# RaghuvirJonnagiri/LatticeBoltzmannSimulations

Measured on AMD Instinct MI355X. Metric: MLUPS (million lattice updates/sec) D2Q9 MRT cavity, higher is better.
Workload: dtype f32

## Files before the change

include/lbm.h:

```cpp
#ifndef LBM_H
#define LBM_H

#include <stddef.h>
#include <stdint.h>

#ifdef __cplusplus
extern "C" {
#endif

#define LBM_ABI_VERSION 4

typedef enum lbm_status {
    LBM_OK = 0,
    LBM_ERR_INVALID = -1,
    LBM_ERR_HIP = -2,
    LBM_ERR_NOMEM = -3,
    LBM_ERR_STATE = -4,
    LBM_ERR_COMM = -5
} lbm_status;

enum { LBM_F32 = 0, LBM_F64 = 1 };
enum { LBM_SRT = 0, LBM_TRT = 1, LBM_MRT = 2 };
enum { LBM_SEM_MRT_PY = 0, LBM_SEM_MRT_GPU = 1,
       LBM_SEM_BOUNCE_BACK = 2 };
// ... 3 lines not shown
       LBM_KERNEL_TB = 3,
       LBM_KERNEL_PUSH = 4,
       LBM_KERNEL_STREAM = 5 };
enum { LBM_LAYOUT_AUTO = 0, LBM_LAYOUT_PLANES = 1, LBM_LAYOUT_ROWS = 2 };
enum { LBM_ARITH_STRICT = 0, LBM_ARITH_FAST = 1, LBM_ARITH_PROMOTED = 2 };
enum { LBM_SIDE_LOW = 0, LBM_SIDE_HIGH = 1 };
enum { LBM_FLAG_NO_DEEP_HALO = 1,
       LBM_FLAG_FRAME_UNFUSED = 2,
       LBM_FLAG_FRAME_FUSED_BATCH = 4,
       LBM_FLAG_NO_FRAME_LDS = 8,
       LBM_FLAG_NT_ON = 16,
       LBM_FLAG_NT_OFF = 32,
       LBM_FLAG_COMM_PRIORITY_OFF = 64,
       LBM_FLAG_EAGER_LAG = 128,
       LBM_FLAG_FRAME_BESIDE_ON = 512,
       LBM_FLAG_FRAME_BESIDE_OFF = 1024,
       LBM_FLAG_FRAME_NARROW = 2048,
       LBM_FLAG_NO_EDGE_FIRST = 4096,
       LBM_FLAG_NO_EDGE_RESERVE = 8192,
       LBM_FLAG_NO_XCD_BANDS = 16384,
       LBM_FLAG_NO_TAIL_TILES = 32768,
       LBM_FLAG_STREAM_WALLS = 65536,
       LBM_FLAG_NO_STREAM_WALLS = 262144,
       LBM_FLAG_STREAM_PAIRS = 131072 };

typedef struct lbm_params {
    int32_t struct_size;
    int32_t nx;
    int32_t ny;
    int32_t y0;
    int32_t ny_local;
    int32_t dtype;
    int32_t collision;
    int32_t semantics;
    int32_t kernel;
    int32_t turb;
    int32_t device;
    int32_t layout;
    int32_t batch;
    int32_t arith;
    int32_t ny_local_min;
    int32_t tb_steps;
    int32_t frame_seg;
    int32_t flags;
    double uLB;
    double omega;
    double omegam;
// ... 56 lines not shown
```

latticeboltzmannsimulations_amd/_lib.py:

```python
import ctypes
import os
import subprocess

_HERE = os.path.dirname(os.path.abspath(__file__))
_CSRC = os.path.join(_HERE, "csrc")
LIB_PATH = os.environ.get("LBM_LIB_PATH", os.path.join(_HERE, "liblbm_hip.so"))
HEADER = os.path.join(os.path.dirname(_HERE), "include", "lbm.h")

HIPCC = os.environ.get("HIPCC", "/opt/rocm/bin/hipcc")
HIPCC_FLAGS = ["--offload-arch=gfx950", "-O3", "-std=c++17", "-ffp-contract=off", "-fPIC", "-shared", "-Wall"]
LINK_FLAGS = ["-ldl"]

LBM_F32, LBM_F64 = 0, 1
LBM_SRT, LBM_TRT, LBM_MRT = 0, 1, 2
LBM_SEM_MRT_PY, LBM_SEM_MRT_GPU, LBM_SEM_BOUNCE_BACK = 0, 1, 2
LBM_KERNEL_AUTO, LBM_KERNEL_GENERIC, LBM_KERNEL_VEC, LBM_KERNEL_TB, LBM_KERNEL_PUSH, LBM_KERNEL_STREAM = 0, 1, 2, 3, 4, 5
LBM_LAYOUT_AUTO, LBM_LAYOUT_PLANES, LBM_LAYOUT_ROWS = 0, 1, 2
LBM_SIDE_LOW, LBM_SIDE_HIGH = 0, 1
LBM_ARITH_STRICT, LBM_ARITH_FAST, LBM_ARITH_PROMOTED = 0, 1, 2
LBM_FLAG_NO_DEEP_HALO, LBM_FLAG_FRAME_UNFUSED, LBM_FLAG_FRAME_FUSED_BATCH, LBM_FLAG_NO_FRAME_LDS = 1, 2, 4, 8
LBM_FLAG_NT_ON, LBM_FLAG_NT_OFF, LBM_FLAG_COMM_PRIORITY_OFF, LBM_FLAG_EAGER_LAG = 16, 32, 64, 128
LBM_FLAG_FRAME_BESIDE_ON, LBM_FLAG_FRAME_BESIDE_OFF, LBM_FLAG_FRAME_NARROW, LBM_FLAG_NO_EDGE_FIRST = 512, 1024, 2048, 4096
LBM_FLAG_NO_EDGE_RESERVE, LBM_FLAG_NO_XCD_BANDS, LBM_FLAG_NO_TAIL_TILES, LBM_FLAG_STREAM_WALLS = 8192, 16384, 32768, 65536
LBM_FLAG_STREAM_PAIRS, LBM_FLAG_NO_STREAM_WALLS = 131072, 262144
ABI_VERSION = 4


class lbm_params(ctypes.Structure):
    _fields_ = [("struct_size", ctypes.c_int32), ("nx", ctypes.c_int32), ("ny", ctypes.c_int32),
                ("y0", ctypes.c_int32), ("ny_local", ctypes.c_int32), ("dtype", ctypes.c_int32),
                ("collision", ctypes.c_int32), ("semantics", ctypes.c_int32), ("kernel", ctypes.c_int32),
                ("turb", ctypes.c_int32), ("device", ctypes.c_int32), ("layout", ctypes.c_int32),
                ("batch", ctypes.c_int32), ("arith", ctypes.c_int32), ("ny_local_min", ctypes.c_int32),
                ("tb_steps", ctypes.c_int32), ("frame_seg", ctypes.c_int32), ("flags", ctypes.c_int32),
                ("uLB", ctypes.c_double), ("omega", ctypes.c_double), ("omegam", ctypes.c_double),
                ("omega_e", ctypes.c_double), ("omega_eps", ctypes.c_double), ("omega_q", ctypes.c_double)]


def sources():
    return [os.path.join(_CSRC, f) for f in sorted(os.listdir(_CSRC)) if f.endswith((".hip", ".hpp"))] + [HEADER]


def build(force=False, verbose=False):
    srcs = sources()
    if not force and os.path.exists(LIB_PATH) and all(os.path.getmtime(LIB_PATH) >= os.path.getmtime(s) for s in srcs):
        return LIB_PATH
    cflags = [f for f in HIPCC_FLAGS if f != "-shared"]
# ... 93 lines not shown
```

latticeboltzmannsimulations_amd/csrc/lbm_host.hpp:

```cpp
#pragma once
#include <hip/hip_runtime.h>
#include <rccl/rccl.h>
#include <dlfcn.h>

#include <algorithm>
#include <chrono>
#include <cstdio>
#include <cstdlib>
#include <cstring>
#include <new>
#include <string>
#include <type_traits>
#include <vector>

#include "../../include/lbm.h"
#include "lbm_inst.hpp"

constexpr int LAT_LAG = 9;
constexpr int NLAT = 10;

enum class Kern { none, tile2, tile, stream, stream_walls, stream_pairs };

struct lbm_ctx {
    lbm_params p{};
// ... 7 lines not shown
    int lag = 0;
    bool lag_valid = false;
    bool lazy_lag = true;
    hipStream_t s_compute = nullptr, s_comm = nullptr;
    hipEvent_t ev_edges = nullptr, ev_halo = nullptr, ev_int = nullptr, ev_go = nullptr, ev_t0 = nullptr, ev_t1 = nullptr;
    void* stage = nullptr;
    size_t stage_bytes = 0;
    double* red_dev = nullptr;
    ncclComm_t comm = nullptr;
    int nranks = 1, rank = 0;
    bool thin_valid = false;
    bool frame_lds = true;
    int frame_seg = 64;
    bool frame_fused = true;
    bool deep_halo = false;
    bool loopback = false;
    bool use_vec = false;
    bool use_nt = false;
    bool push = false;
    Kern kern = Kern::none;
    int edge_rows = 0;
    bool tail_tiles = false;
    bool xcd_bands = true;
    bool edge_reserve = true;
    bool edge_first = true;
    bool frame_wide = true;
    bool frame_beside = false;
    int ncu = 256;
    int tb_steps = 2;
    int tb_f = TB_F;
    int batch = 1;
    long long bstride = 0;
    void* relax_dev = nullptr;
    bool int_stale = false;
    bool edges_pending = false;
    std::string err;
};

namespace lbmhost {

struct rccl_api {
    decltype(&ncclGetUniqueId) GetUniqueId = nullptr;
    decltype(&ncclCommInitRank) CommInitRank = nullptr;
    decltype(&ncclCommDestroy) CommDestroy = nullptr;
    decltype(&ncclGroupStart) GroupStart = nullptr;
    decltype(&ncclGroupEnd) GroupEnd = nullptr;
// ... 110 lines not shown
}
inline int frame_segs(int n, int L) { return (n + L - 1) / L; }
struct StreamPlan { int nstrips, nsegy, H; };

constexpr long long SPIN_US = 3000;
template <typename Q>
bool spin_until_ready(Q&& query) {
    const auto t0 = std::chrono::steady_clock::now();
    for (;;) {
        const hipError_t e = query();
        if (e == hipSuccess) return true;
        if (e != hipErrorNotReady) { (void)hipGetLastError(); return false; }
        if (std::chrono::duration_cast<std::chrono::microseconds>(std::chrono::steady_clock::now() - t0).count() > SPIN_US) return false;
    }
}

inline bool has_neighbour(const lbm_ctx* c, int side) {
    return side == LBM_SIDE_LOW ? c->geo.y0 > 0 : c->geo.y0 + c->geo.ny < c->geo.NY;
}
inline bool is_slab(const lbm_ctx* c) { return has_neighbour(c, LBM_SIDE_LOW) || has_neighbour(c, LBM_SIDE_HIGH); }
inline bool own_transport(const lbm_ctx* c) { return c->comm != nullptr && (c->nranks > 1 || c->loopback); }
inline bool streaming(const lbm_ctx* c) { return c->kern >= Kern::stream; }
inline bool walls_inside(const lbm_ctx* c) { return c->kern >= Kern::stream_walls; }

enum class Route { one_launch, edges_bulk, fused_frame, frame_passes, single_steps };

struct RowBlocks {
    int n = 0;
    char* ptr[Q + 2];
    size_t elems = 0;
};

int ensure_stage(lbm_ctx* c, size_t bytes);
int sync_all(lbm_ctx* c);
int host_to_stage(lbm_ctx* c, const void* host, int host_dtype, int planes);
int stage_to_host(lbm_ctx* c, const void* stage, void* host, int host_dtype, int planes);
bool frame_lds_fits(const lbm_ctx* c, int S, bool deep_rows, int extra = 0, long long budget = FRAME_LDS_BYTES);
int pairs_waves(int S);
StreamPlan plan_stream_on(const lbm_ctx* c, int S, int ncu, long long* cost_out);
StreamPlan plan_stream(const lbm_ctx* c, int S);
bool lag_replayable(const lbm_ctx* c, int S);
int unit_steps(const lbm_ctx* c, int left, bool raw);
Route unit_route(const lbm_ctx* c, int S, bool replay);
std::string validate_params(const lbm_params* p);
lbm_ctx* plan_ctx(const lbm_params* p, int ncu, bool device, std::string& err_out);
int ensure_scratch(lbm_ctx* c, int n);
// ... 27 lines not shown
```

latticeboltzmannsimulations_amd/csrc/lbm_inst.hpp:

```cpp
#pragma once
#include "lbm_stream.hpp"

#define LBM_GPU_VARIANTS(M, R)                                                                                                  \
    M(R, C_SRT, SEM_GPU, false) M(R, C_TRT, SEM_GPU, false) M(R, C_MRT, SEM_GPU, false)                                         \
    M(R, C_MRT_FAST, SEM_GPU, false) M(R, C_SRT_FAST, SEM_GPU, false) M(R, C_TRT_FAST, SEM_GPU, false)                          \
    M(R, C_SRT, SEM_GPU, true) M(R, C_TRT, SEM_GPU, true) M(R, C_MRT, SEM_GPU, true)                                            \
    M(R, C_MRT_FAST, SEM_GPU, true) M(R, C_SRT_FAST, SEM_GPU, true) M(R, C_TRT_FAST, SEM_GPU, true)
#define LBM_PY_VARIANTS(M, R) M(R, C_SRT, SEM_PY, false) M(R, C_TRT, SEM_PY, false) M(R, C_MRT, SEM_PY, false)
#define LBM_BB_VARIANTS(M, R)                                                                                                   \
    M(R, C_SRT, SEM_BB, false) M(R, C_TRT, SEM_BB, false) M(R, C_MRT, SEM_BB, false)                                            \
    M(R, C_MRT_FAST, SEM_BB, false) M(R, C_SRT_FAST, SEM_BB, false) M(R, C_TRT_FAST, SEM_BB, false)
#define LBM_PROM_VARIANTS(M, R)                                                                                                 \
    M(R, C_SRT_PROM, SEM_GPU, false) M(R, C_TRT_PROM, SEM_GPU, false) M(R, C_MRT_PROM, SEM_GPU, false)                          \
    M(R, C_SRT_PROM, SEM_GPU, true) M(R, C_TRT_PROM, SEM_GPU, true) M(R, C_MRT_PROM, SEM_GPU, true)

#define LBM_TILE_ONE(R, COLL, SEM, S, TURB)                                                                                     \
    LBM_X template __global__ void k_stepS_deep<R, COLL, SEM, S, false, TURB>(const R* __restrict__, R* __restrict__, Geo, Relax<R>, Batch<R>, \
                                                                              int, int, int, int, int, FramePtrs<R>, int, int, int, int, int);
#define LBM_TILE_S(R, COLL, SEM, TURB) LBM_TILE_ONE(R, COLL, SEM, 3, TURB) LBM_TILE_ONE(R, COLL, SEM, 4, TURB) LBM_TILE_ONE(R, COLL, SEM, 5, TURB)
#define LBM_STREAM_ONE(R, COLL, SEM, TURB)                                                                                      \
    LBM_X template __global__ void k_stream<R, COLL, SEM, TURB>(const R* __restrict__, R* __restrict__, Geo, Relax<R>, int, int, int, int, int, \
                                                                int, FramePtrs<R>, int, int, int, int, int, int, int, int, int);
#define LBM_STREAMW_ONE(R, COLL, SEM, TURB) \
    LBM_X template __global__ void k_stream_walls<R, COLL, TURB>(const R* __restrict__, R* __restrict__, Geo, Relax<R>, int, int, int, int);
#define LBM_STREAMS_ONE(R, COLL, SEM, TURB)                                                                                     \
    LBM_X template __global__ void k_stream_walls_slab<R, COLL, TURB>(const R* __restrict__, R* __restrict__, Geo, Relax<R>, int, int, int, int, \
                                                                      int, int, int, int, int, int);
#define LBM_STREAMP_ONE(R, COLL, SEM, TURB) \
    LBM_X template __global__ void k_stream_pairs<R, COLL, TURB>(const R* __restrict__, R* __restrict__, Geo, Relax<R>, int, int, int, int);

#define LBM_INST_TILES(R) LBM_GPU_VARIANTS(LBM_TILE_S, R) LBM_PY_VARIANTS(LBM_TILE_S, R)
#define LBM_INST_STREAM(R) LBM_GPU_VARIANTS(LBM_STREAM_ONE, R) LBM_PY_VARIANTS(LBM_STREAM_ONE, R)
#define LBM_INST_STREAMW(R) LBM_GPU_VARIANTS(LBM_STREAMW_ONE, R)
#define LBM_INST_STREAMS(R) LBM_GPU_VARIANTS(LBM_STREAMS_ONE, R)
#define LBM_INST_STREAMP(R) LBM_GPU_VARIANTS(LBM_STREAMP_ONE, R)
#define LBM_INST_TILES_PROM(R) LBM_PROM_VARIANTS(LBM_TILE_S, R)
#define LBM_INST_STREAM_PROM(R) LBM_PROM_VARIANTS(LBM_STREAM_ONE, R) LBM_PROM_VARIANTS(LBM_STREAMW_ONE, R) LBM_PROM_VARIANTS(LBM_STREAMS_ONE, R)
#define LBM_INST_TILES_BB(R) LBM_BB_VARIANTS(LBM_TILE_S, R)
#define LBM_INST_STREAM_BB(R) LBM_BB_VARIANTS(LBM_STREAM_ONE, R)

#ifdef LBM_INST
#define LBM_X
LBM_INST
#else
#define LBM_X extern
LBM_INST_TILES(float) LBM_INST_TILES(double)
LBM_INST_STREAM(float) LBM_INST_STREAM(double)
LBM_INST_STREAMW(float) LBM_INST_STREAMW(double)
LBM_INST_STREAMS(float) LBM_INST_STREAMS(double)
LBM_INST_STREAMP(float) LBM_INST_STREAMP(double)
// ... 5 lines not shown
```

latticeboltzmannsimulations_amd/csrc/lbm_launch.hip:

```cpp
#include "lbm_host.hpp"

namespace lbmhost {

int ensure_scratch(lbm_ctx* c, int n) {
    bool fresh = false;
    for (int i = 2; i < 2 + n && i < LAT_LAG; ++i) {
        if (c->lat[i]) continue;
        hipError_t e = hipMalloc(&c->lat[i], c->lat_bytes);
        if (e != hipSuccess) {
            c->lat[i] = nullptr;
            return fail(c, LBM_ERR_NOMEM, std::string("hipMalloc(scratch lattice of the frame passes): ") + hipGetErrorString(e));
        }
        HIP_TRY(c, hipMemsetAsync(c->lat[i], 0, c->lat_bytes, c->s_compute));
        fresh = true;
    }
    if (fresh) HIP_TRY(c, hipStreamSynchronize(c->s_compute));
    return LBM_OK;
}

int launch_rows(lbm_ctx* c, int from, int to, int row0, int stride, int nrows, hipStream_t s) {
    if (nrows <= 0) return LBM_OK;
    return launch_variant(c, [&](auto v) {
        using VT = decltype(v);
        using R = typename VT::R;
// ... 58 lines not shown
            hipLaunchKernelGGL((k_frame_multi<R, VT::COLL, VT::SEM, VT::TURB, 1024>), dim3(fl.nframe, c->batch), dim3(1024), 0, s, fp, c->geo,
                               relax_of<R>(c->p), batch_of<R>(c), fl.F, S, fl.nsegx, fl.nsegy, lo ? 1 + extra : 0, hi ? 1 + extra : 0, fl.L, 0);
        else
            hipLaunchKernelGGL((k_frame_multi<R, VT::COLL, VT::SEM, VT::TURB, BLK>), dim3(fl.nframe, c->batch), dim3(BLK), 0, s, fp, c->geo,
                               relax_of<R>(c->p), batch_of<R>(c), fl.F, S, fl.nsegx, fl.nsegy, lo ? 1 + extra : 0, hi ? 1 + extra : 0, fl.L,
                               fl.in_lds ? 1 : 0);
    });
}

static int launch_k_stream(lbm_ctx* c, int from, int to, hipStream_t s, int S, const FrameLayout& fl, const StreamPlan& pl, int nseg, int ye,
                           int lo, int hi, int bands, bool xcd_bands) {
    return launch_variant(c, [&](auto v) {
        using VT = decltype(v);
        using R = typename VT::R;
        hipLaunchKernelGGL((k_stream<R, VT::COLL, VT::SEM, VT::TURB>), dim3(fl.nframe + pl.nstrips * nseg), dim3(ST_NT), 0, s, (const R*)c->lat[from],
                           (R*)c->lat[to], c->geo, relax_of<R>(c->p), S, fl.F, c->geo.nx - fl.F, ye, pl.nstrips, pl.H, frame_ptrs<R>(c, from, to, S),
                           fl.nframe, fl.nsegx, fl.nsegy, fl.L, fl.in_lds ? 1 : 0, lo, hi, bands, xcd_bands ? 1 : 0);
    });
}

static int launch_walls(lbm_ctx* c, int from, int to, hipStream_t s, int S, int ybeg, int yend, int bands, int elo, int ehi) {
    const StreamPlan pl = plan_stream(c, S);
    const int xcd = c->xcd_bands ? 1 : 0;
    return launch_variant(c, [&](auto v) {
        using VT = decltype(v);
        using R = typename VT::R;
        if constexpr (VT::SEM == SEM_GPU) {
            const R* src = (const R*)c->lat[from];
            R* dst = (R*)c->lat[to];
            if (is_slab(c))
                hipLaunchKernelGGL((k_stream_walls_slab<R, VT::COLL, VT::TURB>), dim3(pl.nstrips * (bands ? (bands & 1) + (bands >> 1) : pl.nsegy)),
                                   dim3(ST_NT), 0, s, src, dst, c->geo, relax_of<R>(c->p), S, pl.nstrips, pl.H, bands ? 0 : xcd, ybeg, yend, bands,
                                   elo, ehi, bands ? c->tb_f : 0);
            else if constexpr (coll_is_prom(VT::COLL)) {
                hipLaunchKernelGGL((k_stream_walls<R, VT::COLL, VT::TURB>), dim3(pl.nstrips * pl.nsegy), dim3(ST_NT), 0, s, src, dst, c->geo,
                                   relax_of<R>(c->p), S, pl.nstrips, pl.H, xcd);
            } else if (c->kern == Kern::stream_pairs)
                hipLaunchKernelGGL((k_stream_pairs<R, VT::COLL, VT::TURB>), dim3(pl.nstrips * pl.nsegy), dim3(64 * pairs_waves(S)), 0, s, src, dst,
                                   c->geo, relax_of<R>(c->p), S, pl.nstrips, pl.H, xcd);
            else
                hipLaunchKernelGGL((k_stream_walls<R, VT::COLL, VT::TURB>), dim3(pl.nstrips * pl.nsegy), dim3(ST_NT), 0, s, src, dst, c->geo,
                                   relax_of<R>(c->p), S, pl.nstrips, pl.H, xcd);
        }
    });
}

int launch_stream(lbm_ctx* c, int from, int to, hipStream_t s, int S, bool with_frame) {
    const int F = c->tb_f, ny = c->geo.ny;
    if (walls_inside(c)) {
        const bool slab = is_slab(c);
        if (slab == with_frame) return fail(c, LBM_ERR_STATE, "internal: the streaming kernel with the walls inside takes a whole lone lattice or a slab's bulk rows");
        return launch_walls(c, from, to, s, S, has_neighbour(c, LBM_SIDE_LOW) ? F : 0, ny - (has_neighbour(c, LBM_SIDE_HIGH) ? F : 0), 0, 0, 0);
    }
    FrameLayout fl;
    const int rc = frame_layout(c, fl, S, F, ny - F, ST_LDS_BYTES, false, 0, with_frame);
    if (rc) return rc;
    const StreamPlan pl = plan_stream(c, S);
    return launch_k_stream(c, from, to, s, S, fl, pl, pl.nsegy, ny - F, 0, 0, 0, c->xcd_bands);
}

int launch_stream_edges(lbm_ctx* c, int from, int to, hipStream_t s, int S, bool lo, bool hi, int extra) {
    const int elo = lo ? 1 + extra : 0, ehi = hi ? 1 + extra : 0, bands = (lo ? 1 : 0) | (hi ? 2 : 0);
    if (walls_inside(c)) return launch_walls(c, from, to, s, S, 0, 0, bands, elo, ehi);
    const int F = c->tb_f, ny = c->geo.ny;
    FrameLayout fl;
// ... 316 lines not shown
```

latticeboltzmannsimulations_amd/csrc/lbm_plan.hip:

```cpp
#include "lbm_host.hpp"

namespace lbmhost {

bool frame_lds_fits(const lbm_ctx* c, int S, bool deep_rows, int extra, long long budget) {
    if (!c->frame_lds) return false;
    const int F = c->tb_f, L = c->frame_seg, m = S - 1, np = c->p.turb ? Q + 2 : Q;
    const long long row_strip = (long long)(L + 2 * m + 2) * (F + m + (deep_rows ? m + extra : 0) + 2);
    const long long col_strip = (long long)(F + m + 2) * (L + 2 * m + extra + 2);
    return 2 * np * std::max(row_strip, col_strip) * c->es <= budget;
}
int pairs_waves(int S) { return std::min(SP_MAX_WAVES, S + 2); }
StreamPlan plan_stream_on(const lbm_ctx* c, int S, int ncu, long long* cost_out) {
    const bool walls = walls_inside(c);
    const int V = 16 / c->es, Rr = stream_rim(S, V), TXu = 64 * V - 2 * Rr, F = walls ? 0 : c->tb_f;
    const int cols = c->geo.nx - 2 * F;
    const int rows = walls ? c->geo.ny - c->tb_f * ((has_neighbour(c, LBM_SIDE_LOW) ? 1 : 0) + (has_neighbour(c, LBM_SIDE_HIGH) ? 1 : 0))
                           : c->geo.ny - 2 * F;
    StreamPlan best{walls ? stream_walls_strips(c->geo.nx, S, V) : (cols + TXu - 1) / TXu, 1, rows};
    long long best_cost = -1;
    for (int n = 1; n <= 256 && n * 8 <= std::max(rows, 8); ++n) {
        const int H = (rows + n - 1) / n, nseg = (rows + H - 1) / H;
        const long long segs = (long long)best.nstrips * nseg, rounds = (segs + ncu - 1) / ncu;
        long long iters = H + 2 * (S - 1) + ST_WAVES - 1;
        if (c->kern == Kern::stream_pairs) {
// ... 150 lines not shown
    if (p->kernel == LBM_KERNEL_STREAM && !can_stream)
        return "kernel = STREAM takes one lattice (no batch) with nx % (16 / sizeof(real)) == 0, nx >= 64, ny_local >= 64 (on every rank)";
    const long long cells_plan = (long long)p->nx * nyp;
    const bool walls_variant = c->batch == 1 && !slab && p->semantics == LBM_SEM_MRT_GPU && !p->turb && !(p->flags & LBM_FLAG_NO_STREAM_WALLS) &&
                               (p->collision == LBM_MRT || p->collision == LBM_SRT);
    const bool walls_pays = walls_variant && (c->es == 8 ? p->nx >= 1024 && cells_plan >= (1LL << 20)
                                                         : (p->nx >= 4096 && cells_plan >= (2LL << 20)) || (p->nx >= 2048 && cells_plan >= (4LL << 20)));
    const bool stream_pays = walls_pays ||
                             (p->nx >= 2048 ? (slab ? cells_plan >= (1LL << 20) && nyp >= 512 : cells_plan >= ((c->es == 8 ? 4LL : 8LL) << 20))
                                            : cells_plan >= 3072LL * 3072);
    if (!can_stream || !(p->kernel == LBM_KERNEL_STREAM || (p->kernel == LBM_KERNEL_AUTO && stream_pays))) {
        c->kern = can_tb && (p->kernel == LBM_KERNEL_TB || (p->kernel == LBM_KERNEL_AUTO && big)) ? Kern::tile : Kern::none;
        return std::string();
    }
    const int forced = p->flags & (LBM_FLAG_STREAM_WALLS | LBM_FLAG_STREAM_PAIRS);
    const bool walls_ok = c->batch == 1 && p->semantics == LBM_SEM_MRT_GPU && (!slab || !(p->flags & LBM_FLAG_NO_DEEP_HALO));
    bool walls_pay = !p->turb && (p->collision == LBM_MRT || p->collision == LBM_SRT);
    if (walls_ok && walls_pay && device && !forced) {
        dispatch(c->p, [&](auto v) {
            using VT = decltype(v);
            using R = typename VT::R;
            if constexpr (VT::SEM == SEM_GPU) {
                hipFuncAttributes at;
                const void* kern = slab ? reinterpret_cast<const void*>(&k_stream_walls_slab<R, VT::COLL, VT::TURB>)
                                        : reinterpret_cast<const void*>(&k_stream_walls<R, VT::COLL, VT::TURB>);
                if (hipFuncGetAttributes(&at, kern) != hipSuccess || at.localSizeBytes > (p->collision == LBM_SRT ? 128u : 64u))
                    walls_pay = false;
            }
        });
    }
    const bool walls = walls_ok && !(p->flags & LBM_FLAG_NO_STREAM_WALLS) && (walls_pay || forced);
    c->kern = !walls ? Kern::stream : !slab && (p->flags & LBM_FLAG_STREAM_PAIRS) ? Kern::stream_pairs : Kern::stream_walls;
    return std::string();
}

static std::string plan_steps(lbm_ctx* c) {
    const lbm_params* p = &c->p;
    const int nyp = ny_plan(p);
    if (streaming(c)) {
        c->tb_steps = p->tb_steps ? p->tb_steps : ST_MAX_S;
        const int fmin = p->semantics == LBM_SEM_MRT_PY ? 1 : 0;
        c->tb_f = (c->tb_steps + fmin + 3) / 4 * 4;
        while (c->tb_steps > 2 && (p->nx < 2 * c->tb_f + 16 || nyp < 2 * c->tb_f + 16)) {
            c->tb_steps -= 1;
            c->tb_f = (c->tb_steps + fmin + 3) / 4 * 4;
        }
        if (c->kern == Kern::stream_pairs) c->tb_steps = p->tb_steps ? p->tb_steps : 10;
        else if (c->tb_steps > ST_MAX_S)
            return "tb_steps " + std::to_string(ST_MAX_S + 1) + " .. " + std::to_string(SP_MAX_S) + " need the streaming kernel with two rows per wave (a lone lattice, MRT_GPU semantics)";
        if (c->kern == Kern::stream_walls && is_slab(c) && c->tb_steps < 3) c->kern = Kern::stream;
// ... 32 lines not shown
    }
    c->frame_fused = !(p->flags & LBM_FLAG_FRAME_UNFUSED);
    c->frame_lds = !(p->flags & LBM_FLAG_NO_FRAME_LDS);
    c->frame_wide = !(p->flags & LBM_FLAG_FRAME_NARROW);
    if ((c->frame_seg = p->frame_seg)) return;
    const long long cells1 = (long long)p->nx * ny_plan(p) * c->batch;
    c->frame_seg = cells1 <= 512LL * 512 ? 16 : (cells1 <= 1024LL * 1024 ? 32 : 64);
    if (c->kern == Kern::tile && c->frame_fused && !is_slab(c) && c->frame_lds)
        while (c->frame_seg > 16 && !frame_lds_fits(c, c->tb_steps, false, 0, TILE_FRAME_LDS_BYTES)) c->frame_seg -= 8;
    if (streaming(c) && c->frame_lds)
        while (c->frame_seg > 16 && !frame_lds_fits(c, c->tb_steps, false, 1, ST_LDS_BYTES)) c->frame_seg -= 8;
    if (c->frame_beside) {
        const long long per = 2LL * p->nx + 2LL * (ny_plan(p) - 2 * c->tb_f);
        c->frame_seg = std::max(64, (int)(((per + c->ncu - 1) / c->ncu + 7) / 8 * 8));
    }
}

lbm_ctx* plan_ctx(const lbm_params* p, int ncu, bool device, std::string& err_out) {
    lbm_ctx* c = new (std::nothrow) lbm_ctx();
    if (!c) return (err_out = "out of host memory", nullptr);
    c->p = *p;
    c->ncu = ncu;
    plan_geometry(c);
    err_out = plan_kernel(c, device);
    if (err_out.empty()) err_out = plan_steps(c);
    if (!err_out.empty()) return (delete c, nullptr);
    plan_frame(c, device);
    c->edge_first = !(p->flags & LBM_FLAG_NO_EDGE_FIRST);
    c->edge_reserve = !(p->flags & LBM_FLAG_NO_EDGE_RESERVE);
    c->xcd_bands = !(p->flags & LBM_FLAG_NO_XCD_BANDS);
    c->deep_halo = p->semantics == LBM_SEM_MRT_GPU && !(p->flags & LBM_FLAG_NO_DEEP_HALO);
    c->use_nt = (p->flags & LBM_FLAG_NT_ON) ? true : (p->flags & LBM_FLAG_NT_OFF) ? false : (c->lat_bytes > ((size_t)192 << 20));
    c->lazy_lag = !(p->flags & LBM_FLAG_EAGER_LAG);
    return c;
}

}

using namespace lbmhost;

extern "C" {

int lbm_next_unit(const lbm_ctx* c, int steps_left) {
    if (!c || steps_left < 0) return LBM_ERR_INVALID;
    if (c->push) return steps_left > 0 ? 1 : 0;
    return unit_steps(c, steps_left, c->raw[c->cur] != 0);
// ... 62 lines not shown
```

latticeboltzmannsimulations_amd/csrc/lbm_stream.hpp:

```cpp
#pragma once
#include "lbm_kernels.hpp"

constexpr int ST_WAVES = 16;
constexpr int ST_NT = ST_WAVES * 64;
constexpr int ST_MAX_S = ST_WAVES / 2;
constexpr int ST_LDS_BYTES = ST_WAVES * 9 * 1024;

__device__ __forceinline__ int dpp_from_lower(int v) { return __builtin_amdgcn_update_dpp(v, v, 0x138, 0xf, 0xf, false); }
__device__ __forceinline__ int dpp_from_upper(int v) { return __builtin_amdgcn_update_dpp(v, v, 0x130, 0xf, 0xf, false); }
__device__ __forceinline__ float lane_lower(float v) { return __builtin_bit_cast(float, dpp_from_lower(__builtin_bit_cast(int, v))); }
__device__ __forceinline__ float lane_upper(float v) { return __builtin_bit_cast(float, dpp_from_upper(__builtin_bit_cast(int, v))); }
__device__ __forceinline__ double lane_lower(double v) {
    const long long b = __builtin_bit_cast(long long, v);
    const unsigned lo = (unsigned)dpp_from_lower((int)(unsigned)b), hi = (unsigned)dpp_from_lower((int)(unsigned)(b >> 32));
    return __builtin_bit_cast(double, (long long)(((unsigned long long)hi << 32) | lo));
}
__device__ __forceinline__ double lane_upper(double v) {
    const long long b = __builtin_bit_cast(long long, v);
    const unsigned lo = (unsigned)dpp_from_upper((int)(unsigned)b), hi = (unsigned)dpp_from_upper((int)(unsigned)(b >> 32));
    return __builtin_bit_cast(double, (long long)(((unsigned long long)hi << 32) | lo));
}

__device__ __forceinline__ float lane_lower_e(float v, float edge) {
    return __builtin_bit_cast(float, __builtin_amdgcn_update_dpp(__builtin_bit_cast(int, edge), __builtin_bit_cast(int, v), 0x138, 0xf, 0xf, false));
// ... 118 lines not shown
                                         typename VecT<R, V>::type o3, typename VecT<R, V>::type u2, typename VecT<R, V>::type u5,
                                         typename VecT<R, V>::type u6, typename VecT<R, V>::type d4, typename VecT<R, V>::type d7,
                                         typename VecT<R, V>::type d8) {
    in[0] = o0;
    in[2] = u2;
    in[4] = d4;
    if (WALLS) {
        in[1] = shift_from_lower_e<R, V>(o1, (R)0 + o3[1]);
        in[5] = shift_from_lower_e<R, V>(u5, (R)0 + d7[1]);
        in[8] = shift_from_lower_e<R, V>(d8, (R)0 + u6[1]);
        in[3] = shift_from_upper_e<R, V>(o3, (R)0 + o1[V - 2]);
        in[6] = shift_from_upper_e<R, V>(u6, (R)0 + d8[V - 2]);
        in[7] = shift_from_upper_e<R, V>(d7, (R)0 + u5[V - 2]);
    } else {
        in[1] = shift_from_lower<R, V>(o1);
        in[5] = shift_from_lower<R, V>(u5);
        in[8] = shift_from_lower<R, V>(d8);
        in[3] = shift_from_upper<R, V>(o3);
        in[6] = shift_from_upper<R, V>(u6);
        in[7] = shift_from_upper<R, V>(d7);
    }
}

template <typename R, int COLL, bool TURB, bool WALLS = false, bool SLAB = false>
__device__ __forceinline__ void stream_segment(const R* __restrict__ src, R* __restrict__ dst, const Geo& geo, const Relax<R>& w, R* __restrict__ lds,
                                               int S, int xs, int ya, int yb, int xe, int own_lo = 0, int own_hi = 0) {
    constexpr int V = 16 / (int)sizeof(R), ROW = 64 * V;
    typedef typename VecT<R, V>::type T;
    const int wv = __builtin_amdgcn_readfirstlane((int)(threadIdx.x >> 6)), lane = threadIdx.x & 63;
    const int q = ((wv & 7) << 1) | (wv >> 3);
    const int RV = stream_rim(S, V) / V;
    const bool wall_lo = WALLS && (!SLAB || geo.y0 == 0), wall_hi = WALLS && (!SLAB || geo.y0 + geo.ny == geo.NY);
    const int y_first = wall_lo ? max(ya - (S - 1), 0) : ya - (S - 1);
    const int y_end = wall_hi ? min(yb + (S - 1), geo.ny) : yb + (S - 1);
    const int y_lid = wall_lo ? 0 : -(1 << 30), y_bot = wall_hi ? geo.ny - 1 : -(1 << 30);
    const int nb = y_end - y_first;
    const int x0 = xs + lane * V;
    const bool lane_in = x0 < geo.nx;
    const bool lane_out = WALLS ? (x0 >= own_lo && x0 < own_hi) : (lane >= RV && lane < 64 - RV && x0 < xe);
    const bool wl = WALLS && x0 == 0, wr = WALLS && x0 + V == geo.nx;
    const bool side_strip = WALLS && (xs == 0 || xs + ROW >= geo.nx);
    const bool narrow = WALLS && xs + ROW > geo.nx;
    R* const slot_mine = lds + (q * 9) * ROW;
    R* const up_mine = slot_mine + lane * V;
    const R* const up_below = lds + (((q + 1) & (ST_WAVES - 1)) * 9) * ROW + lane * V;
    const R* const down_above = lds + (((q + ST_WAVES - 1) & (ST_WAVES - 1)) * 9 + 3) * ROW + lane * V;

    T in[Q], outv[Q], hq, hr;
#ifdef LBM_EXP_NO_HBM
    auto row_base = [&](const R* p, int k, int y) { return (const char*)(p + ((long long)k * geo.plane + (long long)((y & 63) + GHY) * geo.row)); };
#else
    auto row_base = [&](const R* p, int k, int y) { return (const char*)(p + ((long long)k * geo.plane + (long long)(y + GHY) * geo.row)); };
#endif
    const unsigned lane_off = (unsigned)(GH + x0) * (unsigned)sizeof(R);
    auto cell = [&](const char* base, int dx) {
        unsigned off = lane_off;
        asm volatile("" : "+v"(off));
        return (const R*)(base + (off + (unsigned)(dx * (int)sizeof(R))));
    };
    const unsigned lane_off_ld = WALLS ? (unsigned)(GH + min(x0, max(geo.nx - V, 0))) * (unsigned)sizeof(R) : lane_off;
    auto cell_ld = [&](const char* base, int dx) {
        unsigned off = lane_off_ld;
        asm volatile("" : "+v"(off));
        return (const R*)(base + (off + (unsigned)(dx * (int)sizeof(R))));
    };
    auto load_row = [&](int y, bool exists) {
        if (WALLS) {
            if (exists) {
#pragma unroll
// ... 105 lines not shown
                if (lid) rw_done = *reinterpret_cast<const T*>(st + lane * V);
                kl_done = st[ROW + lane];
                kr_done = st[2 * ROW + lane];
            }
            if (lane_out && y >= ya && y < yb) {
#pragma unroll
                for (int k = 0; k < Q; ++k) vstore<R, V, false>(const_cast<R*>(cell(row_base(dst, k, y), 0)), outv[k]);
                if (TURB) {
                    vstore<R, V, false>(const_cast<R*>(cell(row_base(dst, K_QEQ, y), 0)), hq_done);
                    vstore<R, V, false>(const_cast<R*>(cell(row_base(dst, K_RHO, y), 0)), hr_done);
                }
                if (WALLS && wrow) {
                    if (lid) {
                        vstore<R, V, false>(const_cast<R*>(cell(row_base(dst, 0, -1), 0)), rw_done);
                        if (wl) *const_cast<R*>(cell(row_base(dst, 7, -1), 1)) = kl_done;
                        if (wr) *const_cast<R*>(cell(row_base(dst, 8, -1), V - 2)) = kr_done;
                    } else {
                        if (wl) *const_cast<R*>(cell(row_base(dst, 6, geo.ny), 1)) = kl_done;
                        if (wr) *const_cast<R*>(cell(row_base(dst, 5, geo.ny), V - 2)) = kr_done;
                    }
                }
            }
            if (S > 1) lds_barrier();
            load_row(y_first + b + ST_WAVES, b + ST_WAVES < nb);
            if (S > 1) lds_barrier();
        }
        for (int i = 2 * S; i < ST_WAVES; ++i) lds_barrier();
    };
#pragma unroll
    for (int k = 0; k < Q; ++k) in[k] = T{};
    hq = T{}; hr = T{};
    for (int i = 0; i < q; ++i) lds_barrier();
    load_row(y_first + q, q < nb);
    for (int b = q; b < nb; b += ST_WAVES) {
        const int y = y_first + b;
        if (WALLS && (SLAB ? (y == y_lid || y == y_bot) : (y == 0 || y == geo.ny - 1))) block(b, std::true_type{});
        else block(b, std::false_type{});
    }
}

template <typename R, int COLL, int SEM, bool TURB>
__global__ __launch_bounds__(ST_NT) void k_stream(const R* __restrict__ src, R* __restrict__ dst, Geo geo, Relax<R> w, int S, int F, int xe, int ye,
                                                  int nstrips, int H, FramePtrs<R> fp, int nframe, int nsegx, int nsegy, int seg, int use_lds,
                                                  int lo, int hi, int bands, int xcd_bands) {
    __shared__ __align__(16) R lds[ST_LDS_BYTES / sizeof(R)];
    if ((int)blockIdx.x < nframe) {
        frame_passes<R, COLL, SEM, TURB, ST_NT>(fp, 0, geo, w, F, S, nsegx, nsegy, lo, hi, (int)blockIdx.x, seg, use_lds ? lds : nullptr, bands);
        return;
    }
    constexpr int V = 16 / (int)sizeof(R);
    int b = blockIdx.x - nframe;
    if (xcd_bands) {
        const int per = ((int)gridDim.x - nframe) >> 3;
        if (b < (per << 3)) b = (b & 7) * per + (b >> 3);
    }
    const int strip = b % nstrips, sy = b / nstrips;
    const int R_ = stream_rim(S, V);
// ... 1 lines not shown
    int ya, yb;
    if (bands) {
        const bool top = (bands & 1) && sy == 0;
        if (top) { ya = -(lo > 0 ? lo - 1 : 0); yb = F; }
        else { ya = geo.ny - F; yb = geo.ny + (hi > 0 ? hi - 1 : 0); }
    } else {
        ya = F + sy * H; yb = min(ye, ya + H);
    }
    if (ya >= yb) return;
    stream_segment<R, COLL, TURB>(src, dst, geo, w, lds, S, xs, ya, yb, xe);
}

__host__ __device__ constexpr int stream_walls_strips(int nx, int S, int V) {
    return nx <= 64 * V ? 1 : (nx - 64 * V + (64 * V - 2 * stream_rim(S, V)) - 1) / (64 * V - 2 * stream_rim(S, V)) + 1;
}
template <int V>
__device__ __forceinline__ void walls_strip(const Geo& geo, int S, int strip, int nstrips, int& xs, int& own_lo, int& own_hi) {
    const int R_ = stream_rim(S, V), TXu = 64 * V - 2 * R_;
    xs = min(strip * TXu, max(geo.nx - 64 * V, 0));
    own_lo = strip == 0 ? 0 : strip * TXu + R_;
    own_hi = strip == nstrips - 1 ? geo.nx : (strip + 1) * TXu + R_;
}

template <typename R, int COLL, bool TURB>
__global__ __launch_bounds__(ST_NT) void k_stream_walls(const R* __restrict__ src, R* __restrict__ dst, Geo geo, Relax<R> w, int S, int nstrips, int H,
                                                        int xcd_bands) {
    __shared__ __align__(16) R lds[ST_LDS_BYTES / sizeof(R)];
    constexpr int V = 16 / (int)sizeof(R);
    const int b = xcd_bands ? xcd_band(blockIdx.x, gridDim.x) : (int)blockIdx.x;
    const int strip = b % nstrips, sy = b / nstrips;
    int xs, own_lo, own_hi;
    walls_strip<V>(geo, S, strip, nstrips, xs, own_lo, own_hi);
    const int ya = sy * H, yb = min(geo.ny, ya + H);
    if (ya >= yb) return;
    stream_segment<R, COLL, TURB, true>(src, dst, geo, w, lds, S, xs, ya, yb, 0, own_lo, own_hi);
}
template <typename R, int COLL, bool TURB>
__global__ __launch_bounds__(ST_NT) void k_stream_walls_slab(const R* __restrict__ src, R* __restrict__ dst, Geo geo, Relax<R> w, int S, int nstrips, int H,
                                                             int xcd_bands, int ybeg, int yend, int bands, int lo, int hi, int F) {
    __shared__ __align__(16) R lds[ST_LDS_BYTES / sizeof(R)];
    constexpr int V = 16 / (int)sizeof(R), W = 64 * V;
    int b = blockIdx.x;
    if (xcd_bands) {
        const int per = (int)gridDim.x >> 3;
        if (b < (per << 3)) b = (b & 7) * per + (b >> 3);
    }
    const int strip = b % nstrips, sy = b / nstrips;
    const int R_ = stream_rim(S, V), TXu = W - 2 * R_;
    const int xs = min(strip * TXu, max(geo.nx - W, 0));
    const int own_lo = strip == 0 ? 0 : strip * TXu + R_;
    const int own_hi = strip == nstrips - 1 ? geo.nx : (strip + 1) * TXu + R_;
    int ya, yb;
    if (bands) {
        const bool top = (bands & 1) && sy == 0;
        if (top) { ya = -(lo > 0 ? lo - 1 : 0); yb = F; }
        else { ya = geo.ny - F; yb = geo.ny + (hi > 0 ? hi - 1 : 0); }
    } else {
        ya = ybeg + sy * H; yb = min(yend, ya + H);
    }
    if (ya >= yb) return;
    stream_segment<R, COLL, TURB, true, true>(src, dst, geo, w, lds, S, xs, ya, yb, 0, own_lo, own_hi);
}

constexpr int SP_MAX_WAVES = 12;
constexpr int SP_NT = SP_MAX_WAVES * 64;

constexpr int SP_MAX_S = SP_MAX_WAVES - 2;
constexpr int SP_SLOTS = 12;
constexpr int SP_LDS_BYTES = SP_MAX_WAVES * SP_SLOTS * 1024;

template <typename R, int COLL, bool TURB>
__device__ __forceinline__ void stream_pairs_segment(const R* __restrict__ src, R* __restrict__ dst, const Geo& geo, const Relax<R>& w, R* __restrict__ lds,
                                                     int S, int xs, int ya, int yb, int own_lo, int own_hi) {
    constexpr int V = 16 / (int)sizeof(R), ROW = 64 * V;
    typedef typename VecT<R, V>::type T;
    const int W = (int)(blockDim.x >> 6);
    const int wv = __builtin_amdgcn_readfirstlane((int)(threadIdx.x >> 6)), lane = threadIdx.x & 63;
    const int y_first = max(ya - (S - 1), 0), y_end = min(yb + (S - 1), geo.ny);
    const int nb = y_end - y_first, npairs = (nb + 1) >> 1;
    const int x0 = xs + lane * V;
    const bool lane_out = x0 >= own_lo && x0 < own_hi;
    const bool wl = x0 == 0, wr = x0 + V == geo.nx;
    const bool side_strip = xs == 0 || xs + ROW >= geo.nx;
    const bool narrow = xs + ROW > geo.nx;
// ... 201 lines not shown
```

latticeboltzmannsimulations_amd/solver.py:

```python
import ctypes

import numpy as np

from . import _lib as L

_DT = {np.dtype(np.float32): L.LBM_F32, np.dtype(np.float64): L.LBM_F64}
_COLL = {"SRT": L.LBM_SRT, "TRT": L.LBM_TRT, "MRT": L.LBM_MRT}
_SEM = {"mrt_py": L.LBM_SEM_MRT_PY, "mrt_gpu": L.LBM_SEM_MRT_GPU, "bounce_back": L.LBM_SEM_BOUNCE_BACK}
_KERNEL = {"auto": L.LBM_KERNEL_AUTO, "generic": L.LBM_KERNEL_GENERIC, "vec": L.LBM_KERNEL_VEC, "tb": L.LBM_KERNEL_TB,
           "push": L.LBM_KERNEL_PUSH, "stream": L.LBM_KERNEL_STREAM}
_ARITH = {"strict": L.LBM_ARITH_STRICT, "fast": L.LBM_ARITH_FAST, "promoted": L.LBM_ARITH_PROMOTED}
_LAYOUT = {"auto": L.LBM_LAYOUT_AUTO, "planes": L.LBM_LAYOUT_PLANES, "rows": L.LBM_LAYOUT_ROWS}


def relaxation(Re, ysize, uLB=0.08, omega_eps=1.2, omega_q=1.2):
    nuLB = uLB * ysize / Re
    omega = 2.0 / (6. * nuLB + 1)
    delTRT = 1.0 / 3.5
    omegam = 1.0 / (0.5 + (delTRT / ((1 / omega) - 0.5)))
    return dict(omega=omega, omegam=omegam, omega_e=1.0, omega_eps=omega_eps, omega_q=omega_q)


def _tuning(t):
    t = dict(t or {})
    tb, seg, flags = int(t.pop("tb_steps", 0) or 0), int(t.pop("frame_seg", 0) or 0), 0
    off = {"deep_halo": L.LBM_FLAG_NO_DEEP_HALO, "frame_fused": L.LBM_FLAG_FRAME_UNFUSED, "frame_lds": L.LBM_FLAG_NO_FRAME_LDS,
           "comm_priority": L.LBM_FLAG_COMM_PRIORITY_OFF, "frame_wide": L.LBM_FLAG_FRAME_NARROW, "edge_first": L.LBM_FLAG_NO_EDGE_FIRST,
           "edge_reserve": L.LBM_FLAG_NO_EDGE_RESERVE, "xcd_bands": L.LBM_FLAG_NO_XCD_BANDS,
           "tail_tiles": L.LBM_FLAG_NO_TAIL_TILES}
    on = {"frame_fused_batch": L.LBM_FLAG_FRAME_FUSED_BATCH, "eager_lag": L.LBM_FLAG_EAGER_LAG, "stream_pairs": L.LBM_FLAG_STREAM_PAIRS}
    if "stream_walls" in t:
        flags |= L.LBM_FLAG_STREAM_WALLS if t.pop("stream_walls") else L.LBM_FLAG_NO_STREAM_WALLS
    for k, bit in off.items():
        if not t.pop(k, True):
            flags |= bit
    for k, bit in on.items():
        if t.pop(k, False):
            flags |= bit
    nt = t.pop("nt", None)
    if nt is not None:
        flags |= L.LBM_FLAG_NT_ON if nt else L.LBM_FLAG_NT_OFF
    fb = t.pop("frame_beside", None)
    if fb is not None:
        flags |= L.LBM_FLAG_FRAME_BESIDE_ON if fb else L.LBM_FLAG_FRAME_BESIDE_OFF
    if t:
        raise ValueError(f"unknown tuning switches {sorted(t)}")
    return tb, seg, flags


class CavitySolver:

    def __init__(self, xsize, ysize, Re, RT="MRT", uLB=0.08, semantics="mrt_gpu", dtype=np.float32, turb=0,
# ... 288 lines not shown
```

Baseline: 374,800.

## Split stream-walls workgroup into two independent wave rings for short time units

Adds a SPLIT template variant of the wall-aware streaming kernels. It divides the 16 waves of a workgroup into two independent 8-wave pipelines, each handling half of the row segment with its own LDS region and ring indexing. The variant is used by default when the temporal-blocking depth S is small (2*S fits within the stage limit). The aim is to cut ring fill/drain barriers and idle waves for short units. The cost is more halo rows recomputed per half-segment and extra kernel instantiations, and the variant is dropped if it spills.

```diff
diff --git a/include/lbm.h b/include/lbm.h
--- a/include/lbm.h
+++ b/include/lbm.h
@@ -49,7 +49,8 @@
        LBM_FLAG_NO_TAIL_TILES = 32768,
        LBM_FLAG_STREAM_WALLS = 65536,
        LBM_FLAG_NO_STREAM_WALLS = 262144,
-       LBM_FLAG_STREAM_PAIRS = 131072 };
+       LBM_FLAG_STREAM_PAIRS = 131072,
+       LBM_FLAG_NO_SHORT_SPLIT = 524288 };
 
 typedef struct lbm_params {
     int32_t struct_size;
diff --git a/latticeboltzmannsimulations_amd/_lib.py b/latticeboltzmannsimulations_amd/_lib.py
--- a/latticeboltzmannsimulations_amd/_lib.py
+++ b/latticeboltzmannsimulations_amd/_lib.py
@@ -22,7 +22,7 @@
 LBM_FLAG_NT_ON, LBM_FLAG_NT_OFF, LBM_FLAG_COMM_PRIORITY_OFF, LBM_FLAG_EAGER_LAG = 16, 32, 64, 128
 LBM_FLAG_FRAME_BESIDE_ON, LBM_FLAG_FRAME_BESIDE_OFF, LBM_FLAG_FRAME_NARROW, LBM_FLAG_NO_EDGE_FIRST = 512, 1024, 2048, 4096
 LBM_FLAG_NO_EDGE_RESERVE, LBM_FLAG_NO_XCD_BANDS, LBM_FLAG_NO_TAIL_TILES, LBM_FLAG_STREAM_WALLS = 8192, 16384, 32768, 65536
-LBM_FLAG_STREAM_PAIRS, LBM_FLAG_NO_STREAM_WALLS = 131072, 262144
+LBM_FLAG_STREAM_PAIRS, LBM_FLAG_NO_STREAM_WALLS, LBM_FLAG_NO_SHORT_SPLIT = 131072, 262144, 524288
 ABI_VERSION = 4
 
 
diff --git a/latticeboltzmannsimulations_amd/csrc/lbm_host.hpp b/latticeboltzmannsimulations_amd/csrc/lbm_host.hpp
--- a/latticeboltzmannsimulations_amd/csrc/lbm_host.hpp
+++ b/latticeboltzmannsimulations_amd/csrc/lbm_host.hpp
@@ -53,6 +53,7 @@
     int edge_rows = 0;
     bool tail_tiles = false;
     bool xcd_bands = true;
+    bool short_split = true;
     bool edge_reserve = true;
     bool edge_first = true;
     bool frame_wide = true;
@@ -209,6 +210,7 @@
 inline bool own_transport(const lbm_ctx* c) { return c->comm != nullptr && (c->nranks > 1 || c->loopback); }
 inline bool streaming(const lbm_ctx* c) { return c->kern >= Kern::stream; }
 inline bool walls_inside(const lbm_ctx* c) { return c->kern >= Kern::stream_walls; }
+inline bool split_unit(const lbm_ctx* c, int S) { return c->kern == Kern::stream_walls && c->short_split && S >= 2 && 2 * S <= ST_MAX_S; }
 
 enum class Route { one_launch, edges_bulk, fused_frame, frame_passes, single_steps };
 
diff --git a/latticeboltzmannsimulations_amd/csrc/lbm_inst.hpp b/latticeboltzmannsimulations_amd/csrc/lbm_inst.hpp
--- a/latticeboltzmannsimulations_amd/csrc/lbm_inst.hpp
+++ b/latticeboltzmannsimulations_amd/csrc/lbm_inst.hpp
@@ -21,11 +21,13 @@
 #define LBM_STREAM_ONE(R, COLL, SEM, TURB)                                                                                      \
     LBM_X template __global__ void k_stream<R, COLL, SEM, TURB>(const R* __restrict__, R* __restrict__, Geo, Relax<R>, int, int, int, int, int, \
                                                                 int, FramePtrs<R>, int, int, int, int, int, int, int, int, int);
-#define LBM_STREAMW_ONE(R, COLL, SEM, TURB) \
-    LBM_X template __global__ void k_stream_walls<R, COLL, TURB>(const R* __restrict__, R* __restrict__, Geo, Relax<R>, int, int, int, int);
-#define LBM_STREAMS_ONE(R, COLL, SEM, TURB)                                                                                     \
-    LBM_X template __global__ void k_stream_walls_slab<R, COLL, TURB>(const R* __restrict__, R* __restrict__, Geo, Relax<R>, int, int, int, int, \
-                                                                      int, int, int, int, int, int);
+#define LBM_STREAMW_SPLIT(R, COLL, SEM, TURB, SPLIT) \
+    LBM_X template __global__ void k_stream_walls<R, COLL, TURB, SPLIT>(const R* __restrict__, R* __restrict__, Geo, Relax<R>, int, int, int, int);
+#define LBM_STREAMS_SPLIT(R, COLL, SEM, TURB, SPLIT)                                                                            \
+    LBM_X template __global__ void k_stream_walls_slab<R, COLL, TURB, SPLIT>(const R* __restrict__, R* __restrict__, Geo, Relax<R>, int, int, int, \
+                                                                             int, int, int, int, int, int, int);
+#define LBM_STREAMW_ONE(R, COLL, SEM, TURB) LBM_STREAMW_SPLIT(R, COLL, SEM, TURB, false) LBM_STREAMW_SPLIT(R, COLL, SEM, TURB, true)
+#define LBM_STREAMS_ONE(R, COLL, SEM, TURB) LBM_STREAMS_SPLIT(R, COLL, SEM, TURB, false) LBM_STREAMS_SPLIT(R, COLL, SEM, TURB, true)
 #define LBM_STREAMP_ONE(R, COLL, SEM, TURB) \
     LBM_X template __global__ void k_stream_pairs<R, COLL, TURB>(const R* __restrict__, R* __restrict__, Geo, Relax<R>, int, int, int, int);
 
diff --git a/latticeboltzmannsimulations_amd/csrc/lbm_launch.hip b/latticeboltzmannsimulations_amd/csrc/lbm_launch.hip
--- a/latticeboltzmannsimulations_amd/csrc/lbm_launch.hip
+++ b/latticeboltzmannsimulations_amd/csrc/lbm_launch.hip
@@ -104,25 +104,26 @@
 static int launch_walls(lbm_ctx* c, int from, int to, hipStream_t s, int S, int ybeg, int yend, int bands, int elo, int ehi) {
     const StreamPlan pl = plan_stream(c, S);
     const int xcd = c->xcd_bands ? 1 : 0;
+    const bool split = split_unit(c, S);
     return launch_variant(c, [&](auto v) {
         using VT = decltype(v);
         using R = typename VT::R;
         if constexpr (VT::SEM == SEM_GPU) {
             const R* src = (const R*)c->lat[from];
             R* dst = (R*)c->lat[to];
-            if (is_slab(c))
-                hipLaunchKernelGGL((k_stream_walls_slab<R, VT::COLL, VT::TURB>), dim3(pl.nstrips * (bands ? (bands & 1) + (bands >> 1) : pl.nsegy)),
-                                   dim3(ST_NT), 0, s, src, dst, c->geo, relax_of<R>(c->p), S, pl.nstrips, pl.H, bands ? 0 : xcd, ybeg, yend, bands,
-                                   elo, ehi, bands ? c->tb_f : 0);
-            else if constexpr (coll_is_prom(VT::COLL)) {
-                hipLaunchKernelGGL((k_stream_walls<R, VT::COLL, VT::TURB>), dim3(pl.nstrips * pl.nsegy), dim3(ST_NT), 0, s, src, dst, c->geo,
-                                   relax_of<R>(c->p), S, pl.nstrips, pl.H, xcd);
-            } else if (c->kern == Kern::stream_pairs)
-                hipLaunchKernelGGL((k_stream_pairs<R, VT::COLL, VT::TURB>), dim3(pl.nstrips * pl.nsegy), dim3(64 * pairs_waves(S)), 0, s, src, dst,
-                                   c->geo, relax_of<R>(c->p), S, pl.nstrips, pl.H, xcd);
-            else
-                hipLaunchKernelGGL((k_stream_walls<R, VT::COLL, VT::TURB>), dim3(pl.nstrips * pl.nsegy), dim3(ST_NT), 0, s, src, dst, c->geo,
-                                   relax_of<R>(c->p), S, pl.nstrips, pl.H, xcd);
+            if (is_slab(c)) {
+                auto kern = split ? k_stream_walls_slab<R, VT::COLL, VT::TURB, true> : k_stream_walls_slab<R, VT::COLL, VT::TURB, false>;
+                hipLaunchKernelGGL(kern, dim3(pl.nstrips * (bands ? (bands & 1) + (bands >> 1) : pl.nsegy)), dim3(ST_NT), 0, s, src, dst, c->geo,
+                                   relax_of<R>(c->p), S, pl.nstrips, pl.H, bands ? 0 : xcd, ybeg, yend, bands, elo, ehi, bands ? c->tb_f : 0);
+            } else if (c->kern == Kern::stream_pairs) {
+                if constexpr (!coll_is_prom(VT::COLL))
+                    hipLaunchKernelGGL((k_stream_pairs<R, VT::COLL, VT::TURB>), dim3(pl.nstrips * pl.nsegy), dim3(64 * pairs_waves(S)), 0, s, src,
+                                       dst, c->geo, relax_of<R>(c->p), S, pl.nstrips, pl.H, xcd);
+            } else {
+                auto kern = split ? k_stream_walls<R, VT::COLL, VT::TURB, true> : k_stream_walls<R, VT::COLL, VT::TURB, false>;
+                hipLaunchKernelGGL(kern, dim3(pl.nstrips * pl.nsegy), dim3(ST_NT), 0, s, src, dst, c->geo, relax_of<R>(c->p), S, pl.nstrips,
+                                   pl.H, xcd);
+            }
         }
     });
 }
diff --git a/latticeboltzmannsimulations_amd/csrc/lbm_plan.hip b/latticeboltzmannsimulations_amd/csrc/lbm_plan.hip
--- a/latticeboltzmannsimulations_amd/csrc/lbm_plan.hip
+++ b/latticeboltzmannsimulations_amd/csrc/lbm_plan.hip
@@ -196,10 +196,15 @@
             using R = typename VT::R;
             if constexpr (VT::SEM == SEM_GPU) {
                 hipFuncAttributes at;
-                const void* kern = slab ? reinterpret_cast<const void*>(&k_stream_walls_slab<R, VT::COLL, VT::TURB>)
-                                        : reinterpret_cast<const void*>(&k_stream_walls<R, VT::COLL, VT::TURB>);
-                if (hipFuncGetAttributes(&at, kern) != hipSuccess || at.localSizeBytes > (p->collision == LBM_SRT ? 128u : 64u))
+                const void* kern = slab ? reinterpret_cast<const void*>(&k_stream_walls_slab<R, VT::COLL, VT::TURB, false>)
+                                        : reinterpret_cast<const void*>(&k_stream_walls<R, VT::COLL, VT::TURB, false>);
+                const void* kern_split = slab ? reinterpret_cast<const void*>(&k_stream_walls_slab<R, VT::COLL, VT::TURB, true>)
+                                              : reinterpret_cast<const void*>(&k_stream_walls<R, VT::COLL, VT::TURB, true>);
+                const size_t bound = p->collision == LBM_SRT ? 128u : 64u;
+                if (hipFuncGetAttributes(&at, kern) != hipSuccess || at.localSizeBytes > bound)
                     walls_pay = false;
+                if (hipFuncGetAttributes(&at, kern_split) != hipSuccess || at.localSizeBytes > bound)
+                    c->short_split = false;
             }
         });
     }
@@ -278,6 +283,7 @@
     c->p = *p;
     c->ncu = ncu;
     plan_geometry(c);
+    c->short_split = !(p->flags & LBM_FLAG_NO_SHORT_SPLIT);
     err_out = plan_kernel(c, device);
     if (err_out.empty()) err_out = plan_steps(c);
     if (!err_out.empty()) return (delete c, nullptr);
diff --git a/latticeboltzmannsimulations_amd/csrc/lbm_stream.hpp b/latticeboltzmannsimulations_amd/csrc/lbm_stream.hpp
--- a/latticeboltzmannsimulations_amd/csrc/lbm_stream.hpp
+++ b/latticeboltzmannsimulations_amd/csrc/lbm_stream.hpp
@@ -164,19 +164,25 @@
     }
 }
 
-template <typename R, int COLL, bool TURB, bool WALLS = false, bool SLAB = false>
+template <typename R, int COLL, bool TURB, bool WALLS = false, bool SLAB = false, bool SPLIT = false>
 __device__ __forceinline__ void stream_segment(const R* __restrict__ src, R* __restrict__ dst, const Geo& geo, const Relax<R>& w, R* __restrict__ lds,
                                                int S, int xs, int ya, int yb, int xe, int own_lo = 0, int own_hi = 0) {
     constexpr int V = 16 / (int)sizeof(R), ROW = 64 * V;
+    constexpr int P = SPLIT ? ST_WAVES / 2 : ST_WAVES;
     typedef typename VecT<R, V>::type T;
     const int wv = __builtin_amdgcn_readfirstlane((int)(threadIdx.x >> 6)), lane = threadIdx.x & 63;
-    const int q = ((wv & 7) << 1) | (wv >> 3);
+    const int q = SPLIT ? ((wv & 3) << 1) | ((wv >> 2) & 1) : ((wv & 7) << 1) | (wv >> 3);
+    if constexpr (SPLIT) {
+        const int ym = ya + ((yb - ya + 1) >> 1);
+        if (wv >> 3) { ya = ym; lds += (P * 9) * ROW; }
+        else yb = ym;
+    }
     const int RV = stream_rim(S, V) / V;
     const bool wall_lo = WALLS && (!SLAB || geo.y0 == 0), wall_hi = WALLS && (!SLAB || geo.y0 + geo.ny == geo.NY);
     const int y_first = wall_lo ? max(ya - (S - 1), 0) : ya - (S - 1);
     const int y_end = wall_hi ? min(yb + (S - 1), geo.ny) : yb + (S - 1);
     const int y_lid = wall_lo ? 0 : -(1 << 30), y_bot = wall_hi ? geo.ny - 1 : -(1 << 30);
-    const int nb = y_end - y_first;
+    const int nb = !SPLIT || ya < yb ? y_end - y_first : 0;
     const int x0 = xs + lane * V;
     const bool lane_in = x0 < geo.nx;
     const bool lane_out = WALLS ? (x0 >= own_lo && x0 < own_hi) : (lane >= RV && lane < 64 - RV && x0 < xe);
@@ -185,8 +191,8 @@
     const bool narrow = WALLS && xs + ROW > geo.nx;
     R* const slot_mine = lds + (q * 9) * ROW;
     R* const up_mine = slot_mine + lane * V;
-    const R* const up_below = lds + (((q + 1) & (ST_WAVES - 1)) * 9) * ROW + lane * V;
-    const R* const down_above = lds + (((q + ST_WAVES - 1) & (ST_WAVES - 1)) * 9 + 3) * ROW + lane * V;
+    const R* const up_below = lds + (((q + 1) & (P - 1)) * 9) * ROW + lane * V;
+    const R* const down_above = lds + (((q + P - 1) & (P - 1)) * 9 + 3) * ROW + lane * V;
 
     T in[Q], outv[Q], hq, hr;
 #ifdef LBM_EXP_NO_HBM
@@ -338,17 +344,17 @@
                 }
             }
             if (S > 1) lds_barrier();
-            load_row(y_first + b + ST_WAVES, b + ST_WAVES < nb);
+            load_row(y_first + b + P, b + P < nb);
             if (S > 1) lds_barrier();
         }
-        for (int i = 2 * S; i < ST_WAVES; ++i) lds_barrier();
+        for (int i = 2 * S; i < P; ++i) lds_barrier();
     };
 #pragma unroll
     for (int k = 0; k < Q; ++k) in[k] = T{};
     hq = T{}; hr = T{};
     for (int i = 0; i < q; ++i) lds_barrier();
     load_row(y_first + q, q < nb);
-    for (int b = q; b < nb; b += ST_WAVES) {
+    for (int b = q; b < nb; b += P) {
         const int y = y_first + b;
         if (WALLS && (SLAB ? (y == y_lid || y == y_bot) : (y == 0 || y == geo.ny - 1))) block(b, std::true_type{});
         else block(b, std::false_type{});
@@ -396,7 +402,7 @@
     own_hi = strip == nstrips - 1 ? geo.nx : (strip + 1) * TXu + R_;
 }
 
-template <typename R, int COLL, bool TURB>
+template <typename R, int COLL, bool TURB, bool SPLIT>
 __global__ __launch_bounds__(ST_NT) void k_stream_walls(const R* __restrict__ src, R* __restrict__ dst, Geo geo, Relax<R> w, int S, int nstrips, int H,
                                                         int xcd_bands) {
     __shared__ __align__(16) R lds[ST_LDS_BYTES / sizeof(R)];
@@ -407,9 +413,9 @@
     walls_strip<V>(geo, S, strip, nstrips, xs, own_lo, own_hi);
     const int ya = sy * H, yb = min(geo.ny, ya + H);
     if (ya >= yb) return;
-    stream_segment<R, COLL, TURB, true>(src, dst, geo, w, lds, S, xs, ya, yb, 0, own_lo, own_hi);
-}
-template <typename R, int COLL, bool TURB>
+    stream_segment<R, COLL, TURB, true, false, SPLIT>(src, dst, geo, w, lds, S, xs, ya, yb, 0, own_lo, own_hi);
+}
+template <typename R, int COLL, bool TURB, bool SPLIT>
 __global__ __launch_bounds__(ST_NT) void k_stream_walls_slab(const R* __restrict__ src, R* __restrict__ dst, Geo geo, Relax<R> w, int S, int nstrips, int H,
                                                              int xcd_bands, int ybeg, int yend, int bands, int lo, int hi, int F) {
     __shared__ __align__(16) R lds[ST_LDS_BYTES / sizeof(R)];
@@ -433,7 +439,7 @@
         ya = ybeg + sy * H; yb = min(yend, ya + H);
     }
     if (ya >= yb) return;
-    stream_segment<R, COLL, TURB, true, true>(src, dst, geo, w, lds, S, xs, ya, yb, 0, own_lo, own_hi);
+    stream_segment<R, COLL, TURB, true, true, SPLIT>(src, dst, geo, w, lds, S, xs, ya, yb, 0, own_lo, own_hi);
 }
 
 constexpr int SP_MAX_WAVES = 12;
diff --git a/latticeboltzmannsimulations_amd/solver.py b/latticeboltzmannsimulations_amd/solver.py
--- a/latticeboltzmannsimulations_amd/solver.py
+++ b/latticeboltzmannsimulations_amd/solver.py
@@ -27,7 +27,7 @@
     off = {"deep_halo": L.LBM_FLAG_NO_DEEP_HALO, "frame_fused": L.LBM_FLAG_FRAME_UNFUSED, "frame_lds": L.LBM_FLAG_NO_FRAME_LDS,
            "comm_priority": L.LBM_FLAG_COMM_PRIORITY_OFF, "frame_wide": L.LBM_FLAG_FRAME_NARROW, "edge_first": L.LBM_FLAG_NO_EDGE_FIRST,
            "edge_reserve": L.LBM_FLAG_NO_EDGE_RESERVE, "xcd_bands": L.LBM_FLAG_NO_XCD_BANDS,
-           "tail_tiles": L.LBM_FLAG_NO_TAIL_TILES}
+           "tail_tiles": L.LBM_FLAG_NO_TAIL_TILES, "short_split": L.LBM_FLAG_NO_SHORT_SPLIT}
     on = {"frame_fused_batch": L.LBM_FLAG_FRAME_FUSED_BATCH, "eager_lag": L.LBM_FLAG_EAGER_LAG, "stream_pairs": L.LBM_FLAG_STREAM_PAIRS}
     if "stream_walls" in t:
         flags |= L.LBM_FLAG_STREAM_WALLS if t.pop("stream_walls") else L.LBM_FLAG_NO_STREAM_WALLS
```

After: 379,800, median of 6. 1.01x the previous value.
